# jtdaugherty/flux

Hardware: AMD Instinct MI355X
Metric: Msamples/sec on demo2.yml (fixed spp) (higher is better)
Workload: dtype f64

## Files before the change

flux_amd/csrc/abi.hip:

```cpp
#include <hip/hip_runtime.h>

#include <chrono>
#include <cmath>
#include <cstdarg>
#include <cstdio>
#include <cstring>
#include <memory>
#include <new>
#include <algorithm>
#include <cstdlib>
#include <string>
#include <vector>

#include "../../include/flux_abi.h"
#include "flux_device.h"
#include "flux_tables.h"
#include "flux_math_coeffs.h"

#include "flux_ctx.h"

namespace flux {

thread_local std::string g_last_error;

// ... 51 lines not shown
static void free_ctx(flux_ctx *c) {
    if (!c) return;
    DeviceGuard g(c->device);
    if (c->ev0) (void)hipEventDestroy(c->ev0);
    if (c->ev1) (void)hipEventDestroy(c->ev1);
    (void)hipFree(c->d_shapes);
    (void)hipFree(c->d_mats);
    (void)hipFree(c->d_fscene);
    (void)hipFree(c->d_pix);
    (void)hipFree(c->d_disc);
    (void)hipFree(c->d_hemi);
    (void)hipFree(c->d_gloss);
    (void)hipFree(c->d_glossx);
    (void)hipFree(c->d_gxoff);
    (void)hipFree(c->d_tput);
    (void)hipFree(c->d_setrows);
    (void)hipFree(c->d_rowperm);
    (void)hipFree(c->d_invperm);
    (void)hipFree(c->d_stats);
    (void)hipFree(c->d_tris);
    (void)hipFree(c->d_nodes);
    (void)hipFree(c->d_nodesq);
    (void)hipFree(c->d_arena);
    (void)hipFree(c->d_out);
    delete c;
}

void flux_ctx_destroy(flux_ctx *ctx) { free_ctx(ctx); }

}
// ... 131 lines not shown
        alloc(&c->d_glossx, own * c->N * (size_t)gx_stride);
        alloc_copy(&c->d_gxoff, h.gx_off);
    }
    int tput_bits = 0;
    {
        RenderParams job = h.rp;
        job.nsamp = c->N;
        job.max_depth = (int32_t)c->D;
        const char *tput_env = std::getenv("FLUX_THROUGHPUT_TABLE");
        if (!(tput_env && std::atoi(tput_env) == 0) && tput_table_bytes(job, &tput_bits)) {
            std::vector<double> tput;
            build_tput_table(h, tput_bits, (int)c->D, tput);
            alloc_copy(&c->d_tput, tput);
        }
    }
    alloc(&c->d_setrows, own * sizeof(DevSetRows));
    alloc(&c->d_rowperm, perm_bytes);
    alloc(&c->d_invperm, perm_bytes);
    alloc(&c->d_stats, FLUX_NUM_STATS * sizeof(unsigned long long));
    if (!h.tris.empty()) {
        alloc_copy(&c->d_tris, h.tris);
        alloc_copy(&c->d_nodes, h.nodes);
        alloc_copy(&c->d_nodesq, h.nodesq);
        if (!h.arena.empty()) alloc_copy(&c->d_arena, h.arena);
    }
    if (e == hipSuccess) e = hipMemset(c->d_stats, 0, FLUX_NUM_STATS * sizeof(unsigned long long));
    laps.lap(FLUX_CREATE_MS_UPLOAD);
    if (e == hipSuccess) e = hipEventCreate(&c->ev0);
    if (e == hipSuccess) e = hipEventCreate(&c->ev1);
    laps.lap(FLUX_CREATE_MS_OTHER);
    double tab_ms[3] = {0, 0, 0};
    if (e == hipSuccess)
        e = generate_tables(seed, c->S, c->sets, c->D, c->n, c->H, c->d_pix, c->d_disc, c->d_hemi, c->d_rowperm, c->d_invperm, nullptr, tab_ms);
    if (e == hipSuccess) {
        e = generate_gloss_table(c->d_pix, (size_t)c->sets.count * c->N, c->d_gloss, nullptr);
        if (e == hipSuccess && gx_stride)
            e = generate_glossx_table(c->d_gloss, (size_t)c->sets.count * c->N, h.gx_inv_e1.data(), h.rp.n_gloss_exp, gx_stride / 16,
                                      c->d_glossx, nullptr);
        if (e == hipSuccess) e = hipStreamSynchronize(nullptr);
    }
    laps.lap(FLUX_CREATE_MS_TABLES);
    laps.ms[FLUX_CREATE_MS_TABLES] -= tab_ms[0] + tab_ms[2];
    laps.ms[FLUX_CREATE_MS_ALLOC] += tab_ms[0];
    laps.ms[FLUX_CREATE_MS_FREE] += tab_ms[2];
    if (e == hipSuccess) {
        std::vector<DevSetRows> rows(own, DevSetRows{});
        for (size_t m = 0; m < own; m++) {
            rows[m].pix = c->d_pix + m * c->N;
            rows[m].disc = c->d_disc + m * c->N;
            rows[m].hemi = c->d_hemi + m * c->D * c->N * kHemiDoubles;
            rows[m].gloss = c->d_gloss + m * c->N * 4;
            rows[m].glossx = gx_stride ? c->d_glossx + m * c->N * (size_t)(gx_stride / 16) : nullptr;
        }
// ... 6 lines not shown
    rp = h.rp;
    rp.pixel_denom = 1.0 / (double)((uint64_t)c->n * c->n);
    rp.max_depth = (int32_t)c->D;
    rp.nsamp = c->N;
    rp.shapes = c->d_shapes;
    rp.mats = c->d_mats;
    rp.pix = c->d_pix;
    rp.disc = c->d_disc;
    rp.hemi = c->d_hemi;
    rp.gloss = c->d_gloss;
    rp.glossx = c->d_glossx;
    rp.gx_off = c->d_gxoff;
    rp.gx_stride = gx_stride;
    rp.tput = c->d_tput;
    rp.tput_bits = c->d_tput ? tput_bits : 0;
    rp.set_rows = c->d_setrows;
    rp.rowperm = c->d_rowperm;
    rp.invperm = c->d_invperm;
    for (int k = 0; k < 12; k++) rp.exp2c[k] = fastmath::kExp2Poly[k];
    rp.tris = c->d_tris;
    rp.nodes = c->d_nodes;
    rp.nodesq = c->d_nodesq;
    rp.nodes4 = reinterpret_cast<const DevNode4Q *>(c->d_arena);
    const unsigned char *fs = c->d_fscene;
    rp.fsph = reinterpret_cast<const DevScanSphere *>(fs + h.fs.sph);
    rp.fpln = reinterpret_cast<const DevScanPlane *>(fs + h.fs.pln);
    rp.frec = reinterpret_cast<const DevHitRec *>(fs + h.fs.rec);
    rp.fsph32 = h.filter32 ? reinterpret_cast<const DevScanSphere32 *>(fs + h.fs.s32) : nullptr;
    rp.f32_half = rp.fsph32 && h.f32_half >= 0 ? rp.fsph32 + h.f32_half : nullptr;
    rp.f32_top = rp.fsph32 ? rp.fsph32 + h.f32_top : nullptr;
// ... 462 lines not shown
```

flux_amd/csrc/flux_ctx.h:

```cpp
#pragma once
#include <hip/hip_runtime.h>

#include <chrono>
#include <new>
#include <string>
#include <system_error>

#include "../../include/flux_abi.h"
#include "flux_device.h"
#include "flux_tables.h"
#include "scene_build.h"

namespace flux {

extern thread_local std::string g_last_error;
int fail(int code, const char *fmt, ...) __attribute__((format(printf, 2, 3)));

template <class F> int no_throw(F &&f) {
    try {
        return f();
    } catch (const std::bad_alloc &) {
        return fail(FLUX_E_NOMEM, "host allocation failed");
    } catch (const std::system_error &e) {
        return fail(FLUX_E_NOMEM, "%s", e.what());
// ... 40 lines not shown
struct flux_ctx {
    int device = 0;
    flux::RenderParams rp{};
    uint64_t seed = 0;
    uint32_t n = 0, N = 0, D = 0, S = 0, W = 0, H = 0;
    flux::SetRange sets{0, 1, 0};
    flux::DevShape *d_shapes = nullptr;
    flux::DevMaterial *d_mats = nullptr;
    unsigned char *d_fscene = nullptr;
    double2 *d_pix = nullptr, *d_disc = nullptr;
    double *d_hemi = nullptr;
    double *d_gloss = nullptr;
    double2 *d_glossx = nullptr;
    int32_t *d_gxoff = nullptr;
    double *d_tput = nullptr;
    flux::DevSetRows *d_setrows = nullptr;
    int32_t *d_rowperm = nullptr, *d_invperm = nullptr;
    unsigned long long *d_stats = nullptr;
    bool stats_on = false;
    flux::DevTri *d_tris = nullptr;
    flux::DevNode *d_nodes = nullptr;
    flux::DevNode4A *d_arena = nullptr;
    flux::DevNodeQ *d_nodesq = nullptr;
    flux::BvhInfo bvh{};
    int traversal = FLUX_TRAVERSE_BVH;
    int variant = FLUX_KERNEL_DEFAULT;
    int math = FLUX_MATH_FAST;
    double *d_out = nullptr;
    size_t d_out_doubles = 0;
    hipEvent_t ev0 = nullptr, ev1 = nullptr;
// ... 6 lines not shown
```

flux_amd/csrc/flux_device.h:

```cpp
#pragma once
#include <hip/hip_runtime.h>
#include <stdint.h>

#include "flux_bvh.h"
#include "flux_env_verdict.h"


#ifndef FLUX_UNI_SPHERES
#define FLUX_UNI_SPHERES 2
#endif
#ifndef FLUX_BVH_WIDE_MAX_STACK
#define FLUX_BVH_WIDE_MAX_STACK 48
#endif
#ifndef FLUX_MAX_WAVES_PER_PIXEL
#define FLUX_MAX_WAVES_PER_PIXEL 4
#endif
#ifndef FLUX_MIN_SAMPLES_PER_WAVE
#define FLUX_MIN_SAMPLES_PER_WAVE 4096
#endif

namespace flux {

constexpr int kHemiDoubles = 4;
constexpr double kTMin = 0.0005;
// ... 150 lines not shown
    double fwx, fwy, fwz;
    const double *pxc;
    const DevSetRows *set_rows;
    double exp2c[12];
    const DevScanDisk *fdsk;
    int32_t n_dsk;
    int32_t has_diel;
    const double2 *glossx;
    const int32_t *gx_off;
    int32_t gx_stride, n_gloss_exp;
    const DevScanBox *fbox;
    int32_t n_box;
    int32_t tput_bits;
    const double *tput;
    EnvSphere32 env32;
};

__host__ __device__ inline int hit_records(const RenderParams &p) { return p.n_sph + p.n_pln + p.n_dsk + 6 * p.n_box; }

}
```

flux_amd/csrc/flux_tables.h:

```cpp
#pragma once
#include <hip/hip_runtime.h>
#include <stdint.h>
#include "flux_device.h"
#include "flux_plan.h"

namespace flux {

hipError_t generate_tables(uint64_t seed, uint32_t S, SetRange sets, uint32_t D, uint32_t n, uint32_t H,
                           double2 *pix, double2 *disc, double *hemi, int32_t *rowperm, int32_t *invperm,
                           hipStream_t stream, double *phase_ms = nullptr);
hipError_t generate_sampler_grid(int kind, uint64_t seed, uint32_t n, double *d_xy, double *d_hemi,
                                 hipStream_t stream);
hipError_t generate_gloss_table(const double2 *pix, size_t count, double *gloss, hipStream_t stream);
hipError_t generate_glossx_table(const double *gloss, size_t count, const double *inv_e1, int n, int pad, double2 *out, hipStream_t stream);
hipError_t hemi_to_aos(size_t SD, size_t N, const double *in, double *out, hipStream_t stream);

hipError_t launch_render(const RenderParams &p, int variant, int math, hipStream_t stream);

hipError_t launch_shade_rays(const RenderParams &p, int math, const double *d_rays, int n, int depth, uint32_t set,
                             uint32_t index, double *d_rgb, int *d_hit, double *d_t, hipStream_t stream);

hipError_t launch_fastmath_probe(int fn, const double *a, const double *b, double *out, size_t n,
                                 hipStream_t stream);

}
```

flux_amd/csrc/render.hip:

```cpp
#include "flux_device.h"
#include "flux_plan.h"
#include "flux_tables.h"
#include "flux_math.h"
#include "../../include/flux_abi.h"

#ifndef FLUX_WAVES_PER_EU
#define FLUX_WAVES_PER_EU 3
#endif
#ifndef FLUX_WPE_BVH
#define FLUX_WPE_BVH 4
#endif
#ifndef FLUX_WPE_BVH4
#define FLUX_WPE_BVH4 5
#endif
#ifndef FLUX_BVH4_EARLY_AT
#define FLUX_BVH4_EARLY_AT 48
#endif
#ifndef FLUX_BVH_REFILL_AT
#define FLUX_BVH_REFILL_AT 40
#endif
static_assert(FLUX_BVH4_EARLY_AT >= FLUX_BVH_REFILL_AT,
              "FLUX_BVH4_EARLY_AT must not be below FLUX_BVH_REFILL_AT (render_bvh4_kernel would livelock)");
#ifndef FLUX_BVH_LEAF_NUM
#define FLUX_BVH_LEAF_NUM 2
// ... 80 lines not shown
    double2 v = make_double2(0.0, 0.0);
    if (k < n) {
        const double m_inv_e1 = k == 0 ? e.inv_e1[0] : k == 1 ? e.inv_e1[1] : k == 2 ? e.inv_e1[2] : e.inv_e1[3];
        const double cos_theta = fastmath::fexp2_tab(m_inv_e1 * gloss[t * 4 + 2], fastmath::kExp2Poly);
        const double sin_theta = fastmath::fsqrt(fastmath::ffma(-cos_theta, cos_theta, 1.0));
        v = make_double2(cos_theta, sin_theta);
    }
    out[j] = v;
}
hipError_t generate_glossx_table(const double *gloss, size_t count, const double *inv_e1, int n, int pad, double2 *out, hipStream_t stream) {
    if (count == 0 || n < 1 || n > kGlossExpSlots || pad < n) return count == 0 ? hipSuccess : hipErrorInvalidValue;
    GlossExps e{};
    for (int k = 0; k < n; k++) e.inv_e1[k] = inv_e1[k];
    const size_t threads = count * (size_t)pad;
    glossx_fill_kernel<<<dim3((unsigned)((threads + 255) / 256)), dim3(256), 0, stream>>>(gloss, count, e, n, pad, out);
    return hipGetLastError();
}

hipError_t launch_render(const RenderParams &p, int variant, int math, hipStream_t stream) {
    const LaunchPlan L = plan_render(p, variant, math);
    if (L.kernel < 0) return hipSuccess;
    switch (L.copy) {
        case kCopyStrict: return strict::launch_render_impl(L, p, stream);
        case kCopyFast: return fast::launch_render_impl(L, p, stream);
        case kCopyFastDiel: return fast_diel::launch_render_impl(L, p, stream);
    }
    return hipErrorInvalidValue;
}

hipError_t launch_shade_rays(const RenderParams &p, int math, const double *d_rays, int n, int depth, uint32_t set,
// ... 40 lines not shown
```

flux_amd/csrc/render_body.inc:

```

#undef FLUX_STAGE
#if FLUX_FAST
#define FLUX_STAGE() __builtin_amdgcn_sched_barrier(0)
#else
#define FLUX_STAGE() ((void)0)
#endif

struct Ray {
    double ox, oy, oz, dx, dy, dz;
};

typedef const __attribute__((address_space(4))) RenderParams *ParamsInKernarg;
static_assert(sizeof(DevMaterial) % 16 == 0, "the bounce-weight records behind the materials are read as double2");
__device__ __forceinline__ const RenderParams &relaunder_params(uint32_t tick) {
    ParamsInKernarg p = (ParamsInKernarg)__builtin_amdgcn_kernarg_segment_ptr();
    asm("" : "+s"(p) : "s"(tick));
    return *(const RenderParams *)p;
}

__device__ __forceinline__ unsigned long long ballot64(bool b) { return __builtin_amdgcn_ballot_w64(b); }
__device__ __forceinline__ bool any64(bool b) { return __builtin_amdgcn_ballot_w64(b) != 0ull; }
__device__ __forceinline__ bool all64(bool b) { return __builtin_amdgcn_ballot_w64(!b) == 0ull; }

typedef double flux_d2 __attribute__((ext_vector_type(2)));
// ... 833 lines not shown
    return -1;
#endif
}

__device__ __forceinline__ void path_begin(Path &p) {
    p.depth = 1;
    p.nb = 0;
#if FLUX_FAST
    p.tr = p.tg = p.tb = 1.0;
    p.self = -1;
    p.mat = 0;
#endif
}

#if FLUX_FAST
template <bool STATS, bool TRIS, bool TYP = false, bool FIRST = false, bool UNI = false>
__device__ __forceinline__ void fast_bounce(const RenderParams &P, Path &p, uint32_t set, uint32_t i, int hit, int slot, double t, V3 n,
                                            V3 d, V3 pt, int kind, double fr, double fg, double fb, double m_inv_e1, double ax, double az,
                                            bool unit_n, bool convex, bool is_tri, Stats &st, int cz) {
    (void)cz;
    const bool p_glossy_long = TYP ? false : P.glossy_long != 0;
    const bool p_unit_dirs = TYP ? true : P.unit_dirs != 0;
    const bool p_self_skip = TYP ? true : P.self_skip != 0;
    V3 wi;
    double scale = 1.0;
    const bool matte = kind == kMatMatte;
    FLUX_CENSUS(P, 6 + cz);
#if FLUX_DIEL
    if (!TYP && kind == kMatDielectric) {
        const char *hbase = !TRIS ? reinterpret_cast<const char *>(set_rows_of(P, set).hemi)
                                  : reinterpret_cast<const char *>(P.hemi + (size_t)set * P.max_depth * P.nsamp * 4);
        const double u = gather_global<double>(hbase, ((uint32_t)(p.depth - 1) * P.nsamp + i) * 32u + 16u);
        if (dielectric_dir(n, d, m_inv_e1, u, wi)) {
            if (STATS) st.c[10]++;
            fr = fg = fb = 1.0;
        } else {
            if (STATS) st.c[11]++;
        }
    } else
#endif
    {
        V3 w = n;
// ... 85 lines not shown
            double ww = dot(wi, wi);
            asm("" : "+v"(ww));
            const double ss = __builtin_fma(-0.5, ww, 1.5);
            wi = mk(wi.x * ss, wi.y * ss, wi.z * ss);
        }
    } else if (p_unit_dirs) {
        const double ss = matte ? 1.0 : __builtin_fma(-0.5, dot(wi, wi), 1.5);
        wi = mk(wi.x * ss, wi.y * ss, wi.z * ss);
    }
    if (UNI) {
        p.self = -1;
        if (p_self_skip && convex) p.self = (__double2hiint(t) < 0x408f4000 && dot(n, wi) >= 0.0) ? hit : -1;
    } else {
        p.self = (p_self_skip && convex && __double2hiint(t) < 0x408f4000 && dot(n, wi) >= 0.0) ? hit : -1;
    }
    if (FIRST) {
        p.tr = fr * scale;
        p.tg = fg * scale;
        p.tb = fb * scale;
    } else {
        p.tr *= fr * scale;
        p.tg *= fg * scale;
        p.tb *= fb * scale;
    }
    p.nb++;
    p.depth++;
    p.r.ox = pt.x;
    p.r.oy = pt.y;
    p.r.oz = pt.z;
    p.r.dx = wi.x;
    p.r.dy = wi.y;
    p.r.dz = wi.z;
}

typedef const __attribute__((address_space(4))) DevHitRec *HitRecScalar;
template <bool LDS_SCENE, bool UNI = false>
__device__ __forceinline__ int analytic_hit_fields(const RenderParams &P, const Ray &r, int hit, double t, const char *frec_lds, V3 &n,
                                                   int &kind, bool &unit_n, bool &convex, double &fr, double &fg, double &fb,
                                                   double &m_inv_e1, double &ax, double &az) {
    (void)frec_lds;
    if (UNI) {
        const HitRecScalar Ru = (HitRecScalar)(reinterpret_cast<uintptr_t>(P.frec) + (uint32_t)hit * (uint32_t)sizeof(DevHitRec));
        kind = Ru->mat_kind;
        unit_n = Ru->unit_normal != 0;
        fr = Ru->fr; fg = Ru->fg; fb = Ru->fb; m_inv_e1 = Ru->inv_e1;
        ax = Ru->ax; az = Ru->az;
        const double cx = Ru->cx, cy = Ru->cy, cz = Ru->cz, inv_rad = Ru->inv_rad;
        if (Ru->shape_kind == kShapeSphere) {
            n = mk(((r.ox - cx) + t * r.dx) * inv_rad, ((r.oy - cy) + t * r.dy) * inv_rad, ((r.oz - cz) + t * r.dz) * inv_rad);
            convex = inv_rad > 0.0;
        } else {
            n = mk(cx, cy, cz);
            convex = false;
        }
        return Ru->orig_id;
    }
    const DevHitRec R = *reinterpret_cast<const DevHitRec *>((LDS_SCENE ? frec_lds : reinterpret_cast<const char *>(P.frec)) +
                                                              (uint32_t)hit * (uint32_t)sizeof(DevHitRec));
    kind = R.mat_kind;
    unit_n = R.unit_normal != 0;
    fr = R.fr; fg = R.fg; fb = R.fb; m_inv_e1 = R.inv_e1;
    ax = R.ax; az = R.az;
    const V3 ns = mk(((r.ox - R.cx) + t * r.dx) * R.inv_rad, ((r.oy - R.cy) + t * r.dy) * R.inv_rad,
                     ((r.oz - R.cz) + t * r.dz) * R.inv_rad);
    const bool sph = R.shape_kind == kShapeSphere;
    n = mk(sph ? ns.x : R.cx, sph ? ns.y : R.cy, sph ? ns.z : R.cz);
    convex = sph && R.inv_rad > 0.0;
    return R.orig_id;
}

template <bool STATS, bool TRIS, bool LDS_SCENE = false, bool TYP = false, bool FIRST = false, bool BOUNCE = true, bool FACING = false,
          bool UNI = false>
__device__ __forceinline__ bool shade_hit_fast(const RenderParams &P, Path &p, uint32_t set, uint32_t i, int hit, int slot, double t,
                                               double &Lr, double &Lg, double &Lb, Stats &st, int cz, const char *frec_lds = nullptr,
                                               int facing = 0) {
    (void)frec_lds;
    (void)facing;
    (void)cz;
    int bounce = 0;
    const bool is_tri = TRIS && slot >= 0;
    const V3 d = mk(p.r.dx, p.r.dy, p.r.dz);
    const V3 pt = mk(p.r.ox + t * d.x, p.r.oy + t * d.y, p.r.oz + t * d.z);
    V3 n = mk(0.0, 0.0, 1.0);
    int kind = kMatEmissive;
    bool unit_n = true;
    bool convex = false;
    double fr = 0.0, fg = 0.0, fb = 0.0, m_inv_e1 = 0.0, ax = 0.0, az = 0.0;
    if (hit < 0) {
        Lr = P.bgr;
        Lg = P.bgg;
        Lb = P.bgb;
        if (STATS) st.c[6]++;
    } else {
        if (is_tri) {
            const DevTri &T = P.tris[slot];
            const DevMaterial &Mt = P.mats[T.mat];
            p.mat = T.mat;
            n = mk(T.nx, T.ny, T.nz);
            kind = Mt.kind;
            fr = Mt.fr; fg = Mt.fg; fb = Mt.fb; m_inv_e1 = Mt.inv_e1;
            ax = kind == kMatMatte ? 0.0034 : 0.00424;
            az = kind == kMatMatte ? 0.0071 : 0.00764;
        } else {
            p.mat = analytic_hit_fields<LDS_SCENE, UNI>(P, p.r, hit, t, frec_lds, n, kind, unit_n, convex, fr, fg, fb, m_inv_e1, ax, az);
        }
        if (kind == kMatEmissive) {
            if (STATS) st.c[5]++;
            bool front;
            if (FACING && ballot64(!facing_known(facing)) == 0ull) {
                const DevHitRec &R = *reinterpret_cast<const DevHitRec *>(frec_lds + (uint32_t)hit * (uint32_t)sizeof(DevHitRec));
                front = facing_front(facing, reinterpret_cast<const int *>(&R.inv_rad)[1]);
            } else {
                front = ((n.x * -1.0) * d.x + (n.y * -1.0) * d.y + (n.z * -1.0) * d.z) > 0.0;
            }
            Lr = fr;
            Lg = fg;
            Lb = fb;
            if (ballot64(!front) != 0ull) {
                Lr = front ? fr : 0.0;
                Lg = front ? fg : 0.0;
                Lb = front ? fb : 0.0;
            }
        } else {
            if (UNI) {
                if (BOUNCE) fast_bounce<STATS, TRIS, TYP, FIRST, true>(P, p, set, i, hit, slot, t, n, d, pt, kind, fr, fg, fb, m_inv_e1, ax, az,
                                                                       unit_n, convex, is_tri, st, cz);
                return true;
            }
            bounce = 1;
        }
    }
    if (UNI) return false;
    asm("" : "+v"(bounce));
    if (BOUNCE && bounce) {
        fast_bounce<STATS, TRIS, TYP, FIRST>(P, p, set, i, hit, slot, t, n, d, pt, kind, fr, fg, fb, m_inv_e1, ax, az, unit_n, convex, is_tri, st,
                                            cz);
    }
    return bounce != 0;
}

template <bool STATS, bool TYP>
// ... 604 lines not shown
            }
        }
    }
}

__device__ __forceinline__ double lds_dword_pair(const uint32_t *p) { return __hiloint2double((int)p[1], (int)p[0]); }
__device__ __forceinline__ void lds_dword_pair_store(uint32_t *p, double v) {
    p[0] = (uint32_t)__double2loint(v);
    p[1] = (uint32_t)__double2hiint(v);
}

__device__ __forceinline__ uint32_t *hitq_entry(uint32_t *pool, uint32_t C, uint32_t k) {
    return reinterpret_cast<uint32_t *>(reinterpret_cast<char *>(pool) + __umul24(C - 1u - k, (uint32_t)kHitQBytesPerSlot));
}

template <bool STATS, bool TYP, bool UNIFORM_A>
__device__ __forceinline__ bool shade_primary_hits(const RenderParams &P, Path &p, uint32_t set, uint32_t ia, int hit, double t, double &Lr,
                                                   double &Lg, double &Lb, Stats &st, const char *frec_lds, int uni_a) {
    if (UNIFORM_A) {
        const int hu = __builtin_amdgcn_readfirstlane(hit);
        if (uni_a != 0 && ballot64(hit != hu) == 0ull) {
            FLUX_CENSUS(P, 16);
            return shade_hit_fast<STATS, false, true, TYP, true, true, false, true>(P, p, set, ia, hu, -1, t, Lr, Lg, Lb, st, 3, frec_lds);
        }
    }
    FLUX_CENSUS(P, 17);
    return shade_hit_fast<STATS, false, true, TYP, true>(P, p, set, ia, hit, -1, t, Lr, Lg, Lb, st, 3, frec_lds);
}
constexpr bool split_uniform_a(bool TYP, bool HQ) { return HQ || TYP; }

template <bool STATS, bool MAX32, bool TYP, bool HQ = false>
__global__ __launch_bounds__(64 * FLUX_MAX_WAVES_PER_PIXEL, FLUX_WPE_SPLIT) void render_split_kernel(const RenderParams P0, int hq_cap, int hq_th,
                                                                                                  int hq_bits, int uni_a) {
    (void)hq_cap;
    (void)hq_th;
    (void)hq_bits;
    const RenderParams &P = P0;
    extern __shared__ double lds_stack[];
    __shared__ double part[FLUX_MAX_WAVES_PER_PIXEL][3];
    const int tid = threadIdx.x;
    const uint32_t lane = tid & 63;
    const uint32_t N = P.nsamp;
    const uint32_t K = blockDim.x >> 6, sub = (uint32_t)__builtin_amdgcn_readfirstlane(tid >> 6);
    const uint32_t s_lo = (uint32_t)((uint64_t)N * sub / K), s_hi = (uint32_t)((uint64_t)N * (sub + 1) / K);
// ... 63 lines not shown
                    const uint32_t ic = ia < s_hi ? ia : s_hi - 1u;
                    p.sq = gather_global_d2(pix, ic << 4);
                    p.r = primary_ray_px(P, PX, p.sq, gather_global_d2(disc, ic << 4));
                    if (STATS && valid) {
                        st.c[0]++;
                        st.c[1]++;
                    }
                }
                int hit = -1;
                double t = 0.0;
                scan_shapes_primary<TYP>(P, p.r, cand_p, in_p, in_t0, valid, valid_m, hit, t);
                p.depth = 1;
                if (valid) {
                    double Lr, Lg, Lb;
                    FLUX_CENSUS(P, 2);
                    cont = shade_primary_hits<STATS, TYP, split_uniform_a(TYP, HQ)>(P, p, set_p, ia, hit, t, Lr, Lg, Lb, st, frec_lds, uni_a);
                    if (cont && p.depth > P.max_depth) {
                        cont = false;
                        Lr = Lg = Lb = 0.0;
                        if (STATS) st.c[7]++;
                    }
                    if (!cont) {
                        fold_path(p, nullptr, 0, Lr, Lg, Lb);
                        sr += Lr;
                        sg += Lg;
                        sb += Lb;
                    }
                }
                i = ia;
                ml = (uint32_t)hit;
                if (!cont) p.depth = kDeadDepth;
// ... 165 lines not shown
                {
                    const uint32_t ic = ia < s_hi ? ia : s_hi - 1u;
                    pa.sq = gather_global_d2(pix, ic << 4);
                    pa.r = primary_ray_px(P, PX, pa.sq, gather_global_d2(disc, ic << 4));
                    if (STATS && valid) {
                        st.c[0]++;
                        st.c[1]++;
                    }
                }
                int hit = -1;
                double t = 0.0;
                scan_shapes_primary<TYP>(P, pa.r, cand_p, in_p, in_t0, valid, valid_m, hit, t);
                if (valid) {
                    double Lr, Lg, Lb;
                    FLUX_CENSUS(P, 2);
                    cont = shade_primary_hits<STATS, TYP, split_uniform_a(TYP, HQ)>(P, pa, set_p, ia, hit, t, Lr, Lg, Lb, st, frec_lds, uni_a);
                    if (cont && pa.depth > P.max_depth) {
                        cont = false;
                        Lr = Lg = Lb = 0.0;
                        if (STATS) st.c[7]++;
                    }
                    if (!cont) {
                        fold_path(pa, nullptr, 0, Lr, Lg, Lb);
                        sr += Lr;
                        sg += Lg;
                        sb += Lb;
                    }
                }
                const unsigned long long qmask = ballot64(cont);
                if (cont) {
                    const uint32_t slot = __builtin_amdgcn_mbcnt_hi((uint32_t)(qmask >> 32),
// ... 803 lines not shown
```

flux_amd/csrc/scene_build.cpp:

```cpp
#include "scene_build.h"

#include <algorithm>
#include <cmath>
#include <cstdio>
#include <cstdlib>
#include <cstring>

#include "joining_thread.h"

namespace flux {

namespace {

void normalize3(const double in[3], double out[3]) {
    double len = std::sqrt(in[0] * in[0] + in[1] * in[1] + in[2] * in[2]);
    out[0] = in[0] / len;
    out[1] = in[1] / len;
    out[2] = in[2] / len;
}
void cross3(const double a[3], const double b[3], double o[3]) {
    o[0] = a[1] * b[2] - a[2] * b[1];
    o[1] = a[2] * b[0] - a[0] * b[2];
    o[2] = a[0] * b[1] - a[1] * b[0];
}
// ... 227 lines not shown
        int pairs = ((int)fsph.size() + 1) >> 1;
        const int rem = pairs & 3;
        if (rem == 1 || rem == 2) {
            h.f32_half = pairs - rem;
            pairs -= rem;
        } else if (rem == 3) {
            pairs += 1;
        }
        rp.f32_groups = pairs / 4;
        h.f32_top = pairs;
    }
}

}

void build_tput_table(const HostScene &h, int bits, int max_depth, std::vector<double> &out) {
    const DevHitRec *rec = reinterpret_cast<const DevHitRec *>(h.fscene.data() + h.fs.rec);
    const uint32_t n_rec = (uint32_t)hit_records(h.rp);
    out.assign(((size_t)2 << (bits * (max_depth - 1))) * 3, 0.0);
    for (uint32_t e = 0; e < n_rec; e++) {
        double *t = &out[(size_t)tput_index((uint32_t)bits, e) * 3];
        t[0] = rec[e].fr; t[1] = rec[e].fg; t[2] = rec[e].fb;
    }
    std::vector<uint32_t> heads(n_rec), lists;
    for (uint32_t e = 0; e < n_rec; e++) heads[e] = e;
    for (int n = 2; n < max_depth; n++) {
        const uint32_t head_bits = (uint32_t)(bits * (n - 1));
        lists.clear();
        lists.reserve(heads.size() * n_rec);
        for (uint32_t e = 0; e < n_rec; e++)
// ... 171 lines not shown
```

flux_amd/csrc/scene_build.h:

```cpp
#pragma once
#include <cstddef>
#include <string>
#include <vector>

#include "../../include/flux_abi.h"
#include "flux_device.h"
#include "flux_plan.h"

namespace flux {

struct FsceneLayout {
    size_t sph = 0;
    size_t pln = 0;
    size_t rec = 0;
    size_t s32 = 0;
    size_t ss = 0;
    size_t pxc = 0;
    size_t dsk = 0;
    size_t box = 0;
    size_t bytes = 0;
};
FsceneLayout fscene_layout(size_t n_sph, size_t n_pln, size_t n_dsk, size_t n_box, size_t n_shapes, uint32_t W, uint32_t H);

struct HostScene {
// ... 8 lines not shown
    std::vector<DevNode4A> arena;
    BvhInfo bvh;
    double U[3] = {}, V[3] = {}, W[3] = {};
    RenderParams rp{};
    bool filter32 = false;
    int f32_half = -1;
    int f32_top = 0;
    std::vector<double> gx_inv_e1;
    std::vector<int32_t> gx_off;
};

int build_host_scene(const flux_scene_desc &scene, HostScene &out, std::string &error);

void build_tput_table(const HostScene &h, int bits, int max_depth, std::vector<double> &out);

}
```

Before: 55050.

## Precompute per-record matte lobe tangent frames and load them via scalar path

Adds a device table holding a precomputed orthonormal tangent frame (b1, b2) for each non-sphere hit record, filled by a small kernel at context creation. When a wave-uniform primary hit lands on a matte non-sphere surface, the bounce direction is built from the stored frame and the hemisphere sample, skipping the per-lane cross products, rsqrt and flip logic. The frame is loaded early (typical path) or late (MAX32 path) through scalar constant loads. This costs extra memory and more template instantiations, and the new path also drops the facing-flip and self-skip handling for these hits.

```diff
diff --git a/flux_amd/csrc/abi.hip b/flux_amd/csrc/abi.hip
--- a/flux_amd/csrc/abi.hip
+++ b/flux_amd/csrc/abi.hip
@@ -89,6 +89,7 @@
     (void)hipFree(c->d_glossx);
     (void)hipFree(c->d_gxoff);
     (void)hipFree(c->d_tput);
+    (void)hipFree(c->d_lobe);
     (void)hipFree(c->d_setrows);
     (void)hipFree(c->d_rowperm);
     (void)hipFree(c->d_invperm);
@@ -250,6 +251,9 @@
             alloc_copy(&c->d_tput, tput);
         }
     }
+    std::vector<unsigned char> lobe_entries;
+    const size_t lobe_bytes = lobe_frame_table(h, lobe_entries);
+    if (lobe_bytes) alloc(&c->d_lobe, lobe_bytes);
     alloc(&c->d_setrows, own * sizeof(DevSetRows));
     alloc(&c->d_rowperm, perm_bytes);
     alloc(&c->d_invperm, perm_bytes);
@@ -273,6 +277,8 @@
         if (e == hipSuccess && gx_stride)
             e = generate_glossx_table(c->d_gloss, (size_t)c->sets.count * c->N, h.gx_inv_e1.data(), h.rp.n_gloss_exp, gx_stride / 16,
                                       c->d_glossx, nullptr);
+        if (e == hipSuccess && c->d_lobe)
+            e = generate_lobe_frame_table(reinterpret_cast<const DevHitRec *>(c->d_fscene + h.fs.rec), (int)lobe_entries.size(), c->d_lobe, nullptr);
         if (e == hipSuccess) e = hipStreamSynchronize(nullptr);
     }
     laps.lap(FLUX_CREATE_MS_TABLES);
@@ -309,6 +315,7 @@
     rp.gx_stride = gx_stride;
     rp.tput = c->d_tput;
     rp.tput_bits = c->d_tput ? tput_bits : 0;
+    rp.lobe_frame = c->d_lobe;
     rp.set_rows = c->d_setrows;
     rp.rowperm = c->d_rowperm;
     rp.invperm = c->d_invperm;
diff --git a/flux_amd/csrc/flux_ctx.h b/flux_amd/csrc/flux_ctx.h
--- a/flux_amd/csrc/flux_ctx.h
+++ b/flux_amd/csrc/flux_ctx.h
@@ -78,6 +78,7 @@
     double2 *d_glossx = nullptr;
     int32_t *d_gxoff = nullptr;
     double *d_tput = nullptr;
+    double *d_lobe = nullptr;
     flux::DevSetRows *d_setrows = nullptr;
     int32_t *d_rowperm = nullptr, *d_invperm = nullptr;
     unsigned long long *d_stats = nullptr;
diff --git a/flux_amd/csrc/flux_device.h b/flux_amd/csrc/flux_device.h
--- a/flux_amd/csrc/flux_device.h
+++ b/flux_amd/csrc/flux_device.h
@@ -188,7 +188,9 @@
     int32_t tput_bits;
     const double *tput;
     EnvSphere32 env32;
+    const double *lobe_frame;
 };
+constexpr size_t kLobeFrameBytes = 6 * sizeof(double);
 
 __host__ __device__ inline int hit_records(const RenderParams &p) { return p.n_sph + p.n_pln + p.n_dsk + 6 * p.n_box; }
 
diff --git a/flux_amd/csrc/flux_tables.h b/flux_amd/csrc/flux_tables.h
--- a/flux_amd/csrc/flux_tables.h
+++ b/flux_amd/csrc/flux_tables.h
@@ -13,6 +13,7 @@
                                  hipStream_t stream);
 hipError_t generate_gloss_table(const double2 *pix, size_t count, double *gloss, hipStream_t stream);
 hipError_t generate_glossx_table(const double *gloss, size_t count, const double *inv_e1, int n, int pad, double2 *out, hipStream_t stream);
+hipError_t generate_lobe_frame_table(const DevHitRec *frec, int n_rec, double *out, hipStream_t stream);
 hipError_t hemi_to_aos(size_t SD, size_t N, const double *in, double *out, hipStream_t stream);
 
 hipError_t launch_render(const RenderParams &p, int variant, int math, hipStream_t stream);
diff --git a/flux_amd/csrc/render.hip b/flux_amd/csrc/render.hip
--- a/flux_amd/csrc/render.hip
+++ b/flux_amd/csrc/render.hip
@@ -118,6 +118,35 @@
     for (int k = 0; k < n; k++) e.inv_e1[k] = inv_e1[k];
     const size_t threads = count * (size_t)pad;
     glossx_fill_kernel<<<dim3((unsigned)((threads + 255) / 256)), dim3(256), 0, stream>>>(gloss, count, e, n, pad, out);
+    return hipGetLastError();
+}
+
+__global__ void lobe_frame_fill_kernel(const DevHitRec *__restrict__ frec, int n_rec, double *__restrict__ out) {
+    const int k = (int)(blockIdx.x * blockDim.x + threadIdx.x);
+    if (k >= n_rec) return;
+    const DevHitRec R = frec[k];
+    double b1x = 0.0, b1y = 0.0, b1z = 0.0, b2x = 0.0, b2y = 0.0, b2z = 0.0;
+    if (R.shape_kind != kShapeSphere) {
+        const double nx = R.cx, ny = R.cy, nz = R.cz, ax = R.ax, az = R.az;
+        const double x = fastmath::ffma(-az, ny, nz);
+        const double y = fastmath::ffma(az, nx, -(ax * nz));
+        const double z = fastmath::ffma(ax, ny, -nx);
+        const double dd = fastmath::ffma(z, z, fastmath::ffma(x, x, y * y));
+        const double s = fastmath::frsqrt(dd);
+        b1x = x * s;
+        b1y = y * s;
+        b1z = z * s;
+        b2x = fastmath::ffma(nz, b1y, -(ny * b1z));
+        b2y = fastmath::ffma(nx, b1z, -(nz * b1x));
+        b2z = fastmath::ffma(ny, b1x, -(nx * b1y));
+    }
+    double *o = out + (size_t)k * 6;
+    o[0] = b1x; o[1] = b1y; o[2] = b1z;
+    o[3] = b2x; o[4] = b2y; o[5] = b2z;
+}
+hipError_t generate_lobe_frame_table(const DevHitRec *frec, int n_rec, double *out, hipStream_t stream) {
+    if (n_rec <= 0) return hipSuccess;
+    lobe_frame_fill_kernel<<<dim3((unsigned)((n_rec + 63) / 64)), dim3(64), 0, stream>>>(frec, n_rec, out);
     return hipGetLastError();
 }
 
diff --git a/flux_amd/csrc/render_body.inc b/flux_amd/csrc/render_body.inc
--- a/flux_amd/csrc/render_body.inc
+++ b/flux_amd/csrc/render_body.inc
@@ -871,11 +871,41 @@
 }
 
 #if FLUX_FAST
-template <bool STATS, bool TRIS, bool TYP = false, bool FIRST = false, bool UNI = false>
+constexpr int kLobeOff = 0, kLobeEarly = 1, kLobeLate = 2;
+struct LobeFrameU {
+    double b1x = 0.0, b1y = 0.0, b1z = 0.0, b2x = 0.0, b2y = 0.0, b2z = 0.0;
+    double nx = 0.0, ny = 0.0, nz = 0.0;
+    bool on = false;
+};
+typedef const __attribute__((address_space(4))) double *LobeFrameScalar;
+
+template <bool FIRST>
+__device__ __forceinline__ void advance_path(Path &p, V3 pt, V3 wi, double fr, double fg, double fb, double scale) {
+    if (FIRST) {
+        p.tr = fr * scale;
+        p.tg = fg * scale;
+        p.tb = fb * scale;
+    } else {
+        p.tr *= fr * scale;
+        p.tg *= fg * scale;
+        p.tb *= fb * scale;
+    }
+    p.nb++;
+    p.depth++;
+    p.r.ox = pt.x;
+    p.r.oy = pt.y;
+    p.r.oz = pt.z;
+    p.r.dx = wi.x;
+    p.r.dy = wi.y;
+    p.r.dz = wi.z;
+}
+
+template <bool STATS, bool TRIS, bool TYP = false, bool FIRST = false, bool UNI = false, int LF = kLobeOff>
 __device__ __forceinline__ void fast_bounce(const RenderParams &P, Path &p, uint32_t set, uint32_t i, int hit, int slot, double t, V3 n,
                                             V3 d, V3 pt, int kind, double fr, double fg, double fb, double m_inv_e1, double ax, double az,
-                                            bool unit_n, bool convex, bool is_tri, Stats &st, int cz) {
+                                            bool unit_n, bool convex, bool is_tri, Stats &st, int cz, const LobeFrameU &lf = LobeFrameU()) {
     (void)cz;
+    (void)lf;
     const bool p_glossy_long = TYP ? false : P.glossy_long != 0;
     const bool p_unit_dirs = TYP ? true : P.unit_dirs != 0;
     const bool p_self_skip = TYP ? true : P.self_skip != 0;
@@ -883,6 +913,29 @@
     double scale = 1.0;
     const bool matte = kind == kMatMatte;
     FLUX_CENSUS(P, 6 + cz);
+    if (UNI && !TRIS && LF != kLobeOff && matte && lf.on) {
+        LobeFrameU f = lf;
+        if (LF == kLobeLate) {
+            const LobeFrameScalar F = (LobeFrameScalar)(reinterpret_cast<uintptr_t>(P.lobe_frame) + (uint32_t)hit * (uint32_t)kLobeFrameBytes);
+            f.b1x = F[0]; f.b1y = F[1]; f.b1z = F[2];
+            f.b2x = F[3]; f.b2y = F[4]; f.b2z = F[5];
+        }
+        FLUX_CENSUS(P, 7 + cz);
+        FLUX_CENSUS(P, 18);
+        if (STATS) st.c[2]++;
+        const char *hbase = reinterpret_cast<const char *>(set_rows_of(P, set).hemi);
+        const uint32_t hoff = ((uint32_t)(p.depth - 1) * (uint32_t)P.nsamp + i) * 32u;
+        const double2 hxy = gather_global_d2(hbase, hoff);
+        const double hz = gather_global<double>(hbase, hoff + 16u);
+        const double qx = __builtin_fma(f.b2x, hxy.x, f.b1x * hxy.y);
+        const double qy = __builtin_fma(f.b2y, hxy.x, f.b1y * hxy.y);
+        const double qz = __builtin_fma(f.b2z, hxy.x, f.b1z * hxy.y);
+        V3 wt = mk(__builtin_fma(f.nx, hz, qx), __builtin_fma(f.ny, hz, qy), __builtin_fma(f.nz, hz, qz));
+        if (p_glossy_long && !unit_n) wt = normalize(wt);
+        p.self = -1;
+        advance_path<FIRST>(p, pt, wt, fr, fg, fb, 1.0);
+        return;
+    }
 #if FLUX_DIEL
     if (!TYP && kind == kMatDielectric) {
         const char *hbase = !TRIS ? reinterpret_cast<const char *>(set_rows_of(P, set).hemi)
@@ -998,33 +1051,28 @@
     } else {
         p.self = (p_self_skip && convex && __double2hiint(t) < 0x408f4000 && dot(n, wi) >= 0.0) ? hit : -1;
     }
-    if (FIRST) {
-        p.tr = fr * scale;
-        p.tg = fg * scale;
-        p.tb = fb * scale;
-    } else {
-        p.tr *= fr * scale;
-        p.tg *= fg * scale;
-        p.tb *= fb * scale;
-    }
-    p.nb++;
-    p.depth++;
-    p.r.ox = pt.x;
-    p.r.oy = pt.y;
-    p.r.oz = pt.z;
-    p.r.dx = wi.x;
-    p.r.dy = wi.y;
-    p.r.dz = wi.z;
+    advance_path<FIRST>(p, pt, wi, fr, fg, fb, scale);
 }
 
 typedef const __attribute__((address_space(4))) DevHitRec *HitRecScalar;
-template <bool LDS_SCENE, bool UNI = false>
+template <bool LDS_SCENE, bool UNI = false, int LF = kLobeOff>
 __device__ __forceinline__ int analytic_hit_fields(const RenderParams &P, const Ray &r, int hit, double t, const char *frec_lds, V3 &n,
                                                    int &kind, bool &unit_n, bool &convex, double &fr, double &fg, double &fb,
-                                                   double &m_inv_e1, double &ax, double &az) {
+                                                   double &m_inv_e1, double &ax, double &az, LobeFrameU *lf = nullptr) {
     (void)frec_lds;
     if (UNI) {
         const HitRecScalar Ru = (HitRecScalar)(reinterpret_cast<uintptr_t>(P.frec) + (uint32_t)hit * (uint32_t)sizeof(DevHitRec));
+        if (LF != kLobeOff) {
+            const bool tab = P.lobe_frame != nullptr;
+            if (LF == kLobeEarly) {
+                const LobeFrameScalar F = (LobeFrameScalar)(tab ? reinterpret_cast<uintptr_t>(P.lobe_frame) + (uint32_t)hit * (uint32_t)kLobeFrameBytes
+                                                                : reinterpret_cast<uintptr_t>(Ru));
+                lf->b1x = F[0]; lf->b1y = F[1]; lf->b1z = F[2];
+                lf->b2x = F[3]; lf->b2y = F[4]; lf->b2z = F[5];
+            }
+            lf->nx = Ru->cx; lf->ny = Ru->cy; lf->nz = Ru->cz;
+            lf->on = tab && Ru->shape_kind != kShapeSphere;
+        }
         kind = Ru->mat_kind;
         unit_n = Ru->unit_normal != 0;
         fr = Ru->fr; fg = Ru->fg; fb = Ru->fb; m_inv_e1 = Ru->inv_e1;
@@ -1054,7 +1102,7 @@
 }
 
 template <bool STATS, bool TRIS, bool LDS_SCENE = false, bool TYP = false, bool FIRST = false, bool BOUNCE = true, bool FACING = false,
-          bool UNI = false>
+          bool UNI = false, int LF = kLobeOff>
 __device__ __forceinline__ bool shade_hit_fast(const RenderParams &P, Path &p, uint32_t set, uint32_t i, int hit, int slot, double t,
                                                double &Lr, double &Lg, double &Lb, Stats &st, int cz, const char *frec_lds = nullptr,
                                                int facing = 0) {
@@ -1070,6 +1118,7 @@
     bool unit_n = true;
     bool convex = false;
     double fr = 0.0, fg = 0.0, fb = 0.0, m_inv_e1 = 0.0, ax = 0.0, az = 0.0;
+    LobeFrameU lf;
     if (hit < 0) {
         Lr = P.bgr;
         Lg = P.bgg;
@@ -1086,7 +1135,8 @@
             ax = kind == kMatMatte ? 0.0034 : 0.00424;
             az = kind == kMatMatte ? 0.0071 : 0.00764;
         } else {
-            p.mat = analytic_hit_fields<LDS_SCENE, UNI>(P, p.r, hit, t, frec_lds, n, kind, unit_n, convex, fr, fg, fb, m_inv_e1, ax, az);
+            p.mat = analytic_hit_fields<LDS_SCENE, UNI, UNI ? LF : kLobeOff>(P, p.r, hit, t, frec_lds, n, kind, unit_n, convex, fr, fg, fb, m_inv_e1,
+                                                                             ax, az, &lf);
         }
         if (kind == kMatEmissive) {
             if (STATS) st.c[5]++;
@@ -1107,8 +1157,8 @@
             }
         } else {
             if (UNI) {
-                if (BOUNCE) fast_bounce<STATS, TRIS, TYP, FIRST, true>(P, p, set, i, hit, slot, t, n, d, pt, kind, fr, fg, fb, m_inv_e1, ax, az,
-                                                                       unit_n, convex, is_tri, st, cz);
+                if (BOUNCE) fast_bounce<STATS, TRIS, TYP, FIRST, true, LF>(P, p, set, i, hit, slot, t, n, d, pt, kind, fr, fg, fb, m_inv_e1, ax,
+                                                                           az, unit_n, convex, is_tri, st, cz, lf);
                 return true;
             }
             bounce = 1;
@@ -1743,20 +1793,23 @@
     return reinterpret_cast<uint32_t *>(reinterpret_cast<char *>(pool) + __umul24(C - 1u - k, (uint32_t)kHitQBytesPerSlot));
 }
 
-template <bool STATS, bool TYP, bool UNIFORM_A>
+template <bool STATS, bool TYP, bool UNIFORM_A, int LF>
 __device__ __forceinline__ bool shade_primary_hits(const RenderParams &P, Path &p, uint32_t set, uint32_t ia, int hit, double t, double &Lr,
                                                    double &Lg, double &Lb, Stats &st, const char *frec_lds, int uni_a) {
     if (UNIFORM_A) {
         const int hu = __builtin_amdgcn_readfirstlane(hit);
         if (uni_a != 0 && ballot64(hit != hu) == 0ull) {
             FLUX_CENSUS(P, 16);
-            return shade_hit_fast<STATS, false, true, TYP, true, true, false, true>(P, p, set, ia, hu, -1, t, Lr, Lg, Lb, st, 3, frec_lds);
+            return shade_hit_fast<STATS, false, true, TYP, true, true, false, true, LF>(P, p, set, ia, hu, -1, t, Lr, Lg, Lb, st, 3, frec_lds);
         }
     }
     FLUX_CENSUS(P, 17);
     return shade_hit_fast<STATS, false, true, TYP, true>(P, p, set, ia, hit, -1, t, Lr, Lg, Lb, st, 3, frec_lds);
 }
 constexpr bool split_uniform_a(bool TYP, bool HQ) { return HQ || TYP; }
+constexpr int split_lobe_frames(bool MAX32, bool TYP, bool HQ) {
+    return !split_uniform_a(TYP, HQ) ? kLobeOff : TYP ? kLobeEarly : MAX32 ? kLobeLate : kLobeOff;
+}
 
 template <bool STATS, bool MAX32, bool TYP, bool HQ = false>
 __global__ __launch_bounds__(64 * FLUX_MAX_WAVES_PER_PIXEL, FLUX_WPE_SPLIT) void render_split_kernel(const RenderParams P0, int hq_cap, int hq_th,
@@ -1850,7 +1903,7 @@
                 if (valid) {
                     double Lr, Lg, Lb;
                     FLUX_CENSUS(P, 2);
-                    cont = shade_primary_hits<STATS, TYP, split_uniform_a(TYP, HQ)>(P, p, set_p, ia, hit, t, Lr, Lg, Lb, st, frec_lds, uni_a);
+                    cont = shade_primary_hits<STATS, TYP, split_uniform_a(TYP, HQ), split_lobe_frames(MAX32, TYP, HQ)>(P, p, set_p, ia, hit, t, Lr, Lg, Lb, st, frec_lds, uni_a);
                     if (cont && p.depth > P.max_depth) {
                         cont = false;
                         Lr = Lg = Lb = 0.0;
@@ -2046,7 +2099,7 @@
                 if (valid) {
                     double Lr, Lg, Lb;
                     FLUX_CENSUS(P, 2);
-                    cont = shade_primary_hits<STATS, TYP, split_uniform_a(TYP, HQ)>(P, pa, set_p, ia, hit, t, Lr, Lg, Lb, st, frec_lds, uni_a);
+                    cont = shade_primary_hits<STATS, TYP, split_uniform_a(TYP, HQ), split_lobe_frames(MAX32, TYP, HQ)>(P, pa, set_p, ia, hit, t, Lr, Lg, Lb, st, frec_lds, uni_a);
                     if (cont && pa.depth > P.max_depth) {
                         cont = false;
                         Lr = Lg = Lb = 0.0;
diff --git a/flux_amd/csrc/scene_build.cpp b/flux_amd/csrc/scene_build.cpp
--- a/flux_amd/csrc/scene_build.cpp
+++ b/flux_amd/csrc/scene_build.cpp
@@ -265,6 +265,17 @@
 
 }
 
+size_t lobe_frame_table(const HostScene &h, std::vector<unsigned char> &has_entry) {
+    has_entry.clear();
+    const char *env = std::getenv("FLUX_LOBE_FRAMES");
+    const size_t n_rec = (size_t)hit_records(h.rp);
+    if ((env && std::atoi(env) == 0) || n_rec == 0) return 0;
+    const DevHitRec *rec = reinterpret_cast<const DevHitRec *>(h.fscene.data() + h.fs.rec);
+    has_entry.resize(n_rec);
+    for (size_t k = 0; k < n_rec; k++) has_entry[k] = rec[k].shape_kind != kShapeSphere;
+    return n_rec * kLobeFrameBytes;
+}
+
 void build_tput_table(const HostScene &h, int bits, int max_depth, std::vector<double> &out) {
     const DevHitRec *rec = reinterpret_cast<const DevHitRec *>(h.fscene.data() + h.fs.rec);
     const uint32_t n_rec = (uint32_t)hit_records(h.rp);
diff --git a/flux_amd/csrc/scene_build.h b/flux_amd/csrc/scene_build.h
--- a/flux_amd/csrc/scene_build.h
+++ b/flux_amd/csrc/scene_build.h
@@ -46,4 +46,6 @@
 
 void build_tput_table(const HostScene &h, int bits, int max_depth, std::vector<double> &out);
 
+size_t lobe_frame_table(const HostScene &h, std::vector<unsigned char> &has_entry);
+
 }
diff --git a/profiles/r13_lobe_frames/frame_block_after.s b/profiles/r13_lobe_frames/frame_block_after.s
--- /dev/null
+++ b/profiles/r13_lobe_frames/frame_block_after.s
@@ -0,0 +1,89 @@
+.LBB25_139:
+	s_cmp_gt_i32 s74, -1
+	s_cbranch_scc0 .LBB25_211
+	s_load_dwordx2 s[46:47], s[70:71], 0x188
+	s_waitcnt lgkmcnt(0)
+	s_load_dwordx2 s[6:7], s[70:71], 0x320
+	s_mul_i32 s75, s74, 0x60
+	s_mul_i32 s8, s74, 48
+	v_mul_f64 v[38:39], v[12:13], v[44:45]
+	s_add_u32 s4, s46, s75
+	s_addc_u32 s5, s47, 0
+	s_load_dwordx2 s[48:49], s[46:47], s75 offset:0x40
+	s_load_dwordx4 s[16:19], s[46:47], s75 offset:0x0
+	s_load_dwordx2 s[42:43], s[46:47], s75 offset:0x10
+	s_waitcnt lgkmcnt(0)
+	s_cmp_lg_u64 s[6:7], 0
+	s_cselect_b64 s[2:3], -1, 0
+	s_add_u32 s8, s6, s8
+	s_addc_u32 s9, s7, 0
+	s_and_b64 s[6:7], s[2:3], exec
+	v_mul_f64 v[42:43], v[14:15], v[44:45]
+	v_mul_f64 v[48:49], v[16:17], v[44:45]
+	s_mov_b64 s[44:45], 0
+	s_cselect_b32 s51, s9, s5
+	s_cselect_b32 s50, s8, s4
+	s_cmp_lg_u32 s48, 0
+	v_mov_b64_e32 v[8:9], s[16:17]
+	v_mov_b64_e32 v[10:11], s[18:19]
+	v_mov_b64_e32 v[40:41], s[42:43]
+	s_cbranch_scc1 .LBB25_142
+	s_load_dwordx2 s[4:5], s[4:5], 0x18
+	v_add_f64 v[0:1], v[20:21], -s[16:17]
+	v_add_f64 v[0:1], v[38:39], v[0:1]
+	v_add_f64 v[2:3], v[22:23], -s[18:19]
+	v_add_f64 v[2:3], v[42:43], v[2:3]
+	s_waitcnt lgkmcnt(0)
+	v_mul_f64 v[8:9], v[0:1], s[4:5]
+	v_add_f64 v[0:1], v[24:25], -s[42:43]
+	v_add_f64 v[0:1], v[48:49], v[0:1]
+	v_mul_f64 v[10:11], v[2:3], s[4:5]
+	v_mul_f64 v[40:41], v[0:1], s[4:5]
+	v_cmp_gt_f64_e64 s[44:45], s[4:5], 0
+.LBB25_142:
+	s_load_dwordx4 s[12:15], s[46:47], s75 offset:0x20
+	s_load_dwordx2 s[40:41], s[46:47], s75 offset:0x30
+	s_cmp_lg_u32 s49, 1
+	s_mov_b64 s[26:27], -1
+	s_cbranch_scc0 .LBB25_244
+	s_cmp_lg_u32 s48, 0
+	s_load_dwordx8 s[4:11], s[50:51], 0x0
+	s_load_dwordx4 s[20:23], s[50:51], 0x20
+	s_cselect_b64 s[50:51], -1, 0
+	s_and_b64 s[2:3], s[2:3], s[50:51]
+	s_cmp_lg_u32 s49, 0
+	s_cselect_b64 s[50:51], -1, 0
+	s_cmp_eq_u32 s49, 0
+	s_cselect_b64 s[76:77], -1, 0
+	s_and_b64 s[2:3], s[76:77], s[2:3]
+	s_andn2_b64 vcc, exec, s[2:3]
+	s_cbranch_vccz .LBB25_245
+.LBB25_245:
+	s_cbranch_execnz .LBB25_263
+	s_branch .LBB25_264
+.LBB25_263:
+	s_load_dwordx2 s[2:3], s[38:39], 0x10
+	v_lshlrev_b32_e32 v4, 5, v18
+	v_mov_b32_e32 v63, -1
+	s_waitcnt lgkmcnt(0)
+	global_load_dwordx4 v[0:3], v4, s[2:3]
+	s_nop 0
+	global_load_dwordx2 v[4:5], v4, s[2:3] offset:16
+	s_waitcnt vmcnt(1)
+	v_mul_f64 v[6:7], s[4:5], v[2:3]
+	v_mul_f64 v[46:47], s[6:7], v[2:3]
+	v_mul_f64 v[50:51], s[8:9], v[2:3]
+	v_fmac_f64_e32 v[6:7], s[10:11], v[0:1]
+	v_fmac_f64_e32 v[46:47], s[20:21], v[0:1]
+	v_fmac_f64_e32 v[50:51], s[22:23], v[0:1]
+	s_waitcnt vmcnt(0)
+	v_fmac_f64_e32 v[6:7], s[16:17], v[4:5]
+	v_fmac_f64_e32 v[46:47], s[18:19], v[4:5]
+	v_fmac_f64_e32 v[50:51], s[42:43], v[4:5]
+.LBB25_264:
+	v_add_f64 v[0:1], v[20:21], v[38:39]
+	v_add_f64 v[2:3], v[22:23], v[42:43]
+	v_add_f64 v[4:5], v[24:25], v[48:49]
+	s_waitcnt lgkmcnt(0)
+	s_mov_b32 s4, 2
+	s_cbranch_execnz .LBB25_268
diff --git a/profiles/r13_lobe_frames/frame_block_before.s b/profiles/r13_lobe_frames/frame_block_before.s
--- /dev/null
+++ b/profiles/r13_lobe_frames/frame_block_before.s
@@ -0,0 +1,184 @@
+.LBB24_139:
+	s_cmp_gt_i32 s20, -1
+	s_cbranch_scc0 .LBB24_225
+	s_load_dwordx2 s[16:17], s[70:71], 0x188
+	s_mul_i32 s21, s20, 0x60
+	v_mul_f64 v[46:47], v[12:13], v[44:45]
+	v_mul_f64 v[48:49], v[14:15], v[44:45]
+	v_mul_f64 v[50:51], v[16:17], v[44:45]
+	s_waitcnt lgkmcnt(0)
+	s_load_dwordx2 s[18:19], s[16:17], s21 offset:0x40
+	s_load_dwordx4 s[4:7], s[16:17], s21 offset:0x0
+	s_load_dwordx2 s[2:3], s[16:17], s21 offset:0x10
+	s_mov_b64 s[12:13], 0
+	s_waitcnt lgkmcnt(0)
+	s_cmp_lg_u32 s18, 0
+	v_mov_b64_e32 v[38:39], s[4:5]
+	v_mov_b64_e32 v[40:41], s[6:7]
+	v_mov_b64_e32 v[42:43], s[2:3]
+	s_cbranch_scc1 .LBB24_142
+	s_add_u32 s10, s16, s21
+	s_addc_u32 s11, s17, 0
+	s_load_dwordx2 s[10:11], s[10:11], 0x18
+	v_add_f64 v[0:1], v[20:21], -s[4:5]
+	v_add_f64 v[0:1], v[46:47], v[0:1]
+	v_add_f64 v[2:3], v[22:23], -s[6:7]
+	v_add_f64 v[2:3], v[48:49], v[2:3]
+	s_waitcnt lgkmcnt(0)
+	v_mul_f64 v[38:39], v[0:1], s[10:11]
+	v_add_f64 v[0:1], v[24:25], -s[2:3]
+	v_add_f64 v[0:1], v[50:51], v[0:1]
+	v_mul_f64 v[40:41], v[2:3], s[10:11]
+	v_mul_f64 v[42:43], v[0:1], s[10:11]
+	v_cmp_gt_f64_e64 s[12:13], s[10:11], 0
+.LBB24_142:
+	s_load_dwordx4 s[4:7], s[16:17], s21 offset:0x20
+	s_load_dwordx2 s[10:11], s[16:17], s21 offset:0x30
+	s_cmp_lg_u32 s19, 1
+	s_mov_b64 s[2:3], -1
+	s_cbranch_scc0 .LBB24_258
+	s_cmp_lg_u32 s19, 0
+	s_cselect_b64 s[14:15], -1, 0
+	s_cmp_eq_u32 s19, 0
+	v_mov_b64_e32 v[6:7], v[38:39]
+	v_mov_b64_e32 v[8:9], v[40:41]
+	v_mov_b64_e32 v[10:11], v[42:43]
+	s_cbranch_scc1 .LBB24_145
+	v_mul_f64 v[0:1], v[14:15], v[40:41]
+	v_fmac_f64_e32 v[0:1], v[12:13], v[38:39]
+	v_fmac_f64_e32 v[0:1], v[16:17], v[42:43]
+	v_mul_f64 v[2:3], v[38:39], v[0:1]
+	v_fma_f64 v[6:7], -2.0, v[2:3], v[12:13]
+	v_mul_f64 v[2:3], v[40:41], v[0:1]
+	v_mul_f64 v[0:1], v[42:43], v[0:1]
+	v_fma_f64 v[8:9], -2.0, v[2:3], v[14:15]
+	v_fma_f64 v[10:11], -2.0, v[0:1], v[16:17]
+.LBB24_145:
+	s_cmp_eq_u32 s19, 2
+	s_cbranch_scc1 .LBB24_153
+	v_lshlrev_b32_e32 v52, 5, v18
+	v_mov_b32_e32 v53, 0
+	s_and_b64 vcc, exec, s[14:15]
+	s_cbranch_vccz .LBB24_269
+	s_load_dwordx2 s[18:19], s[70:71], 0x2e0
+	s_load_dwordx4 s[24:27], s[38:39], 0x18
+	s_load_dword s22, s[70:71], 0x2e8
+	s_lshl_b32 s23, s20, 2
+	s_waitcnt lgkmcnt(0)
+	s_load_dword s18, s[18:19], s23 offset:0x0
+	v_lshl_add_u64 v[0:1], s[24:25], 0, v[52:53]
+	global_load_dwordx4 v[54:57], v[0:1], off
+	s_waitcnt lgkmcnt(0)
+	v_mov_b32_e32 v0, s18
+	v_mad_u32_u24 v0, s22, v18, v0
+	global_load_dwordx4 v[0:3], v0, s[26:27]
+	s_waitcnt vmcnt(0)
+	v_mul_f64 v[4:5], v[54:55], v[2:3]
+	v_mul_f64 v[2:3], v[56:57], v[2:3]
+	s_cbranch_execnz .LBB24_149
+.LBB24_148:
+	s_load_dwordx2 s[18:19], s[38:39], 0x10
+	s_waitcnt lgkmcnt(0)
+	v_lshl_add_u64 v[2:3], s[18:19], 0, v[52:53]
+	global_load_dwordx2 v[0:1], v[2:3], off offset:16
+	s_nop 0
+	global_load_dwordx4 v[2:5], v[2:3], off
+.LBB24_149:
+	s_load_dwordx4 s[24:27], s[16:17], s21 offset:0x50
+	s_mov_b32 s16, 0
+	s_mov_b32 s17, 0x3fd80000
+	s_andn2_b64 vcc, exec, s[14:15]
+	s_waitcnt lgkmcnt(0)
+	v_mul_f64 v[54:55], s[24:25], v[10:11]
+	v_fma_f64 v[54:55], s[26:27], v[6:7], -v[54:55]
+	v_fma_f64 v[52:53], -s[26:27], v[8:9], v[10:11]
+	v_mul_f64 v[58:59], v[54:55], v[54:55]
+	v_fma_f64 v[56:57], s[24:25], v[8:9], -v[6:7]
+	v_fmac_f64_e32 v[58:59], v[52:53], v[52:53]
+	v_fmac_f64_e32 v[58:59], v[56:57], v[56:57]
+	v_rsq_f64_e32 v[60:61], v[58:59]
+	s_nop 0
+	v_mul_f64 v[58:59], v[58:59], -v[60:61]
+	v_fma_f64 v[58:59], v[58:59], v[60:61], 1.0
+	v_fma_f64 v[62:63], v[58:59], s[16:17], 0.5
+	v_mul_f64 v[58:59], v[60:61], v[58:59]
+	v_fmac_f64_e32 v[60:61], v[58:59], v[62:63]
+	v_mul_f64 v[52:53], v[52:53], v[60:61]
+	v_mul_f64 v[58:59], v[54:55], v[60:61]
+	v_mul_f64 v[60:61], v[56:57], v[60:61]
+	v_mul_f64 v[54:55], v[8:9], v[60:61]
+	v_fma_f64 v[56:57], v[10:11], v[58:59], -v[54:55]
+	v_mul_f64 v[54:55], v[10:11], v[52:53]
+	v_fma_f64 v[62:63], v[6:7], v[60:61], -v[54:55]
+	v_mul_f64 v[54:55], v[6:7], v[58:59]
+	v_fma_f64 v[64:65], v[8:9], v[52:53], -v[54:55]
+	s_waitcnt vmcnt(0)
+	v_mul_f64 v[54:55], v[52:53], v[4:5]
+	v_fmac_f64_e32 v[54:55], v[56:57], v[2:3]
+	v_mul_f64 v[56:57], v[58:59], v[4:5]
+	v_mul_f64 v[58:59], v[60:61], v[4:5]
+	v_fmac_f64_e32 v[56:57], v[62:63], v[2:3]
+	v_fmac_f64_e32 v[58:59], v[64:65], v[2:3]
+	v_fma_f64 v[2:3], v[6:7], v[0:1], v[54:55]
+	v_fma_f64 v[4:5], v[8:9], v[0:1], v[56:57]
+	v_fma_f64 v[52:53], v[10:11], v[0:1], v[58:59]
+	s_cbranch_vccnz .LBB24_152
+	v_mul_f64 v[60:61], v[40:41], v[4:5]
+	v_fmac_f64_e32 v[60:61], v[38:39], v[2:3]
+	v_fmac_f64_e32 v[60:61], v[42:43], v[52:53]
+	v_cmp_gt_f64_e32 vcc, 0, v[60:61]
+	s_cbranch_vccz .LBB24_152
+	v_mul_f64 v[6:7], v[6:7], v[0:1]
+	v_mul_f64 v[8:9], v[8:9], v[0:1]
+	v_mul_f64 v[0:1], v[10:11], v[0:1]
+	v_add_f64 v[0:1], v[0:1], -v[58:59]
+	v_cndmask_b32_e32 v53, v53, v1, vcc
+	v_cndmask_b32_e32 v52, v52, v0, vcc
+	v_add_f64 v[0:1], v[8:9], -v[56:57]
+	v_cndmask_b32_e32 v5, v5, v1, vcc
+	v_cndmask_b32_e32 v4, v4, v0, vcc
+	v_add_f64 v[0:1], v[6:7], -v[54:55]
+	v_cndmask_b32_e32 v3, v3, v1, vcc
+	v_cndmask_b32_e32 v2, v2, v0, vcc
+.LBB24_152:
+	v_mov_b64_e32 v[10:11], v[52:53]
+	v_mov_b64_e32 v[8:9], v[4:5]
+	v_mov_b64_e32 v[6:7], v[2:3]
+.LBB24_153:
+	s_andn2_b64 vcc, exec, s[14:15]
+	s_cbranch_vccnz .LBB24_155
+	v_mul_f64 v[0:1], v[8:9], v[8:9]
+	v_fmac_f64_e32 v[0:1], v[6:7], v[6:7]
+	v_mov_b32_e32 v2, 0
+	v_fmac_f64_e32 v[0:1], v[10:11], v[10:11]
+	v_mov_b32_e32 v3, 0x3ff80000
+	s_nop 0
+	v_fmac_f64_e32 v[2:3], -0.5, v[0:1]
+	v_mul_f64 v[6:7], v[6:7], v[2:3]
+	v_mul_f64 v[8:9], v[8:9], v[2:3]
+	v_mul_f64 v[10:11], v[10:11], v[2:3]
+.LBB24_155:
+	s_andn2_b64 vcc, exec, s[12:13]
+	v_mov_b32_e32 v63, -1
+	s_cbranch_vccnz .LBB24_161
+	s_mov_b32 s12, 0x408f4000
+	v_cmp_gt_i32_e32 vcc, s12, v45
+	v_mov_b32_e32 v63, -1
+	s_and_saveexec_b64 s[12:13], vcc
+	s_cbranch_execz .LBB24_160
+	v_mul_f64 v[0:1], v[40:41], v[8:9]
+	v_fmac_f64_e32 v[0:1], v[38:39], v[6:7]
+	v_fmac_f64_e32 v[0:1], v[42:43], v[10:11]
+	v_cmp_le_f64_e32 vcc, 0, v[0:1]
+	v_mov_b32_e32 v63, -1
+	s_and_saveexec_b64 s[14:15], vcc
+	v_mov_b32_e32 v63, s20
+	s_or_b64 exec, exec, s[14:15]
+.LBB24_160:
+	s_or_b64 exec, exec, s[12:13]
+.LBB24_161:
+	v_add_f64 v[0:1], v[20:21], v[46:47]
+	v_add_f64 v[2:3], v[22:23], v[48:49]
+	v_add_f64 v[4:5], v[24:25], v[50:51]
+	s_mov_b32 s14, 2
+	s_branch .LBB24_262
```

Measured after the change: 55960 (median of 6 runs). 1.6% higher.
